# shamanDevel/IsosurfaceSuperresolution

Hardware: AMD Instinct MI355X
Metric: frames/sec (render+4×SR) at 256³→1080p, 1/2/4/8 GPU; PSNR vs ref (higher is better)
Workload: dtype f32 (fp32 tensors and accumulation; each product as three fp16 MFMAs on split operands, error vs fp64 = the fp32 kernels')

## Files before the change

### include/isr_sr_kernels.h

```cpp
#ifndef ISR_SR_KERNELS_H
#define ISR_SR_KERNELS_H

#ifdef __cplusplus
extern "C" {
#endif

#define ISR_ACT_NONE 0
#define ISR_ACT_RELU 1
#define ISR_ACT_LEAKY 2
#define ISR_ACT_GATE 3

int isrConvCinPad(int Cin);
int isrConvCoutPad(int Cout);

int isrConvPrepareWeights(const float* w, float* wprep, int Cout, int Cin, int transpose_flip, void* stream);

int isrConv3x3Forward(const float* x, const float* wprep, const float* bias, const float* residual, float* y,
                      int N, int Cin, int H, int W, int Cout, int act, float slope, int upsample2x, void* stream);

int isrConv3x3ForwardStrided(const float* x, const float* wprep, const float* bias, const float* residual, float* y,
                             int N, int Cin, int H, int W, int Cout, int act, float slope, int upsample2x,
                             long long xPlane, long long xImage, long long yPlane, long long yImage,
                             long long rPlane, long long rImage, void* stream);

int isrConvSmallCinPad(int Cin);
long long isrConvSmallWeightFloats(int Cin);
int isrConvSmallPrepare(const float* w, const float* bias, float* w8, float* bias8, int Cout, int Cin, void* stream);
int isrConv3x3SmallCout(const float* x, const float* w8, const float* bias8, const float* residual, float* y,
                        int N, int Cin, int H, int W, int Cout, int act, float slope, void* stream);
int isrConv3x3SmallCoutStrided(const float* x, const float* w8, const float* bias8, const float* residual, float* y,
                               int N, int Cin, int H, int W, int Cout, int act, float slope,
                               long long xPlane, long long xImage, void* stream);

long long isrConvSplitWeightBytes(int Cin, int Cout);
int isrConvSplitPrepare(const float* w, void* wq, int Cout, int Cin, void* stream);
int isrConvSplitPrepareManyMax(void);
int isrConvSplitPrepareMany(int n, const float* const* w, void* const* wqForward, void* const* wqBackward, const int* cout, const int* cin, void* stream);
int isrConv3x3ForwardSplit(const float* x, const void* wq, const float* bias, const float* residual, float* y,
                           int N, int Cin, int H, int W, int Cout, int act, float slope, int upsample2x,
                           long long xPlane, long long xImage, long long yPlane, long long yImage,
                           long long rPlane, long long rImage, void* stream);

long long isrConvF16WeightBytes(int Cin, int Cout);
int isrConvF16Prepare(const float* w, void* wq, int Cout, int Cin, void* stream);
int isrConv3x3ForwardF16(const float* x, const void* wq, const float* bias, const float* residual, float* y,
                         int N, int Cin, int H, int W, int Cout, int act, float slope, int upsample2x,
                         long long xPlane, long long xImage, long long yPlane, long long yImage,
                         long long rPlane, long long rImage, void* stream);
int isrConvBf16Prepare(const float* w, void* wq, int Cout, int Cin, void* stream);
int isrConv3x3ForwardBf16(const float* x, const void* wq, const float* bias, const float* residual, float* y,
                          int N, int Cin, int H, int W, int Cout, int act, float slope, int upsample2x,
                          long long xPlane, long long xImage, long long yPlane, long long yImage,
                          long long rPlane, long long rImage, void* stream);
int isrConvF16SupportsUpsample(long long x_address, int Win, long long xPlane, long long xImage);

long long isrConvWeightGradWorkspace(int N, int Cin, int H, int W, int Cout);
int isrConv3x3WeightGrad(const float* x, const float* gz, float* dw, float* db, void* workspace,
                         int N, int Cin, int H, int W, int Cout, void* stream);

int isrConvWeightGradMaxSegments(void);
int isrConv3x3WeightGradSegments(const float* const* xs, const float* const* gzs, int segments, float* dw, float* db, void* workspace,
                                 int N, int Cin, int H, int W, int Cout, void* stream);
int isrConv3x3WeightGradSegmentsSplit(const float* const* xs, const float* const* gzs, int segments, float* dw, float* db, void* workspace,
                                      int N, int Cin, int H, int W, int Cout, void* stream);
void isrSetMaxSlots(void* words, int capacity);
int isrTakeMaxSlotWords(void);
int isrConv3x3WeightGradSegmentsSplitMax(const float* const* xs, const float* const* gzs, const void* const* gzmax, int maxWords, int segments,
                                         float* dw, float* db, void* workspace, int N, int Cin, int H, int W, int Cout, void* stream);
void isrSetWeightGradAccumulate(int bits);
int isrConv3x3WeightGradSegmentsBf16(const float* const* xs, const float* const* gzs, int segments, float* dw, float* db, void* workspace,
                                     int N, int Cin, int H, int W, int Cout, void* stream);

int isrUpsample2xForward(const float* x, float* y, long long planes, int h, int w, void* stream);
int isrUpsample2xBackward(const float* gy, float* gx, long long planes, int h, int w, void* stream);

int isrReconResidualForward(const float* y, const float* x, float* out, int N, int Cout, int Cin, int k, int h, int w, void* stream);
int isrReconResidualBackward(const float* gy, float* gx, int N, int Cout, int Cin, int k, int h, int w, void* stream);

long long isrLossUnshadedWorkspace(void);
int isrLossUnshadedForward(const float* gt, const float* pred, const float* prev, int N, int H, int W, int pad,
                           const float* weights15, unsigned enabled, const float* shading12, float ao_strength, int inverse_ao,
                           void* workspace, float* values16, void* stream);
int isrLossUnshadedBackward(const float* gt, const float* pred, const float* prev, int N, int H, int W, int pad,
                            const float* weights15, unsigned enabled, const float* shading12, float ao_strength, int inverse_ao,
                            const float* gvalues16, float* gpred, float* gprev, void* stream);

int isrRecurrentInputForward(const float* prev_raw, const float* input, const float* flow, float* net_input, float* warped,
                             int B, int h, int w, long long inputBatchStride, long long flowBatchStride, void* stream);
int isrRecurrentInputBackward(const float* prev_raw, const float* flow, const float* g_net_input, const float* g_warped,
                              float* scratch, float* g_prev_raw, int B, int h, int w, long long flowBatchStride, void* stream);

int isrAdamFlatStep(float* params, const float* grads, float* exp_avg, float* exp_avg_sq, long long n, const float* lr_dev, float lr,
                    float beta1, float beta2, float eps, float* step, void* stream);

int isrActBackward(const float* gy, const float* y, float* gz, long long count, int act, float slope, void* stream);

int isrAssembleInput(const float* gbuffer_hwc12, const float* flow_filled, const float* prev_high, float* net_input,
                     int h, int w, int init_mode, int ao_inverted, void* stream);
int isrAssembleInputRows(const float* gbuffer_hwc12, const float* flow_filled, const float* prev_high, float* net_input,
                         int h, int w, int init_mode, int ao_inverted, int row0, int row1, void* stream);
int isrAssembleInputRect(const float* gbuffer_hwc12, const float* flow_filled, const float* prev_high, float* net_input,
                         int h, int w, int init_mode, int ao_inverted, int row0, int row1, int col0, int col1, void* stream);
int isrAssembleInputPacked(const float* gbuffer_hwc12, const float* flow_filled, const float* prev_high, float* net_input,
                           int h, int w, int init_mode, int ao_inverted, void* trunk_workspace, void* stream);

long long isrFlowFillWorkspace(int h, int w);
int isrFlowFill(const float* gbuffer_hwc12, float* flow_out, void* workspace, int h, int w, void* stream);
int isrFlowFillEx(const float* gbuffer_hwc12, float* flow_out, void* workspace, int h, int w, int threads, void* stream);
int isrFlowFillOneSupported(int h, int w);
int isrFlowFillOne(const float* gbuffer_hwc12, float* flow_out, void* workspace, int h, int w, void* stream);
void isrSetFlowFillErrorWord(unsigned* word);

int isrFinishFrame(const float* raw, const float* net_input, float* next_prev, float* rgb, int h, int w,
                   const float* shading24, int exponent, float ao_strength, int inverse_ao, int enable_specular, void* stream);

int isrConvSmallFinishFrame(const float* x, const float* w8, const float* bias8, const float* net_input, float* next_prev, float* rgb,
                            int Cin, int h, int w, long long xPlane, const float* shading24, int exponent, float ao_strength,
                            int inverse_ao, int enable_specular, void* stream);

int isrConv3x3ForwardSplitPacked(const float* x, const void* wq, const float* bias, void* ps, int Cin, int H, int W, int Cout,
                                 int act, float slope, int upsample2x, long long xPlane, long long psPlane, void* stream);

int isrConv3x3ForwardSplitFromPacked(const void* xps, const void* wq, const float* bias, const float* residual, void* y, int packed_out,
                                     int Cin, int H, int W, int Cout, int act, float slope, long long xpsPlane, long long yPlane, long long rPlane,
                                     void* stream);

int isrTrunkDataflowMaxTiles(void);
long long isrTrunkDataflowWorkspaceBytes(int cin0, int H, int W);
int isrTrunkDataflowSupported(const float* x, int cin0, int H, int W, long long xPlane, long long plane);
int isrTrunkDataflow(const float* x, int cin0, long long xPlane, float* y, long long plane, const void* const* wq,
                     const float* const* bias, int nblocks, int H, int W, void* workspace, void* stream);
int isrTrunkDataflowInputLayout(int cin0, int H, int W, long long* offsets3, int* groups0, int* tiles);
int isrTrunkDataflowPrepacked(int cin0, float* y, long long plane, const void* const* wq, const float* const* bias, int nblocks, int H, int W,
                              void* workspace, void* stream);
void isrSetTrunkErrorWord(unsigned* word);

int isrResBlockSmallSupported(int N, int H, int W);
int isrResBlockSmall(const float* x, const void* wa, const float* ba, const float* gate, const void* wb, const float* bb, float* z, float* y,
                     int N, int H, int W, void* zmax, void* ymax, void* stream);

long long isrResBlockSplitWorkspaceBytes(void);
int isrResBlockSplitSupported(const float* x, int H, int W, long long xPlane, long long yPlane);
int isrResBlockSplit(const float* x, const void* wq1, const float* bias1, const void* wq2, const float* bias2, float* y, void* workspace,
                     int H, int W, long long xPlane, long long yPlane, void* stream);

long long isrConvTailWeightBytes(void);
long long isrConvTailWorkspaceBytes(int h, int w);
int isrConvTailPrepare(const float* w8, void* wz, void* stream);
int isrConvTailSupported(const float* x, int h, int w, long long xPlane);
int isrConvTailFinishFrame(const float* x, const void* wq6, const float* bias6, const void* wz, const float* bias8, void* workspace,
                           const float* net_input, float* next_prev, float* rgb, int h, int w, long long xPlane,
                           const float* shading24, int exponent, float ao_strength, int inverse_ao, int enable_specular, void* stream);
int isrConvTailFinishFramePacked(const void* xps, const void* wq6, const float* bias6, const void* wz, const float* bias8, void* workspace,
                                 const float* net_input, float* next_prev, float* rgb, int h, int w, long long xpsPlane,
                                 const float* shading24, int exponent, float ao_strength, int inverse_ao, int enable_specular, void* stream);

long long isrConvUpsPhaseWeightBytes(void);
long long isrConvUpsPhaseScratchBytes(void);
int isrConvUpsPhasePrepare(const float* w, void* wq, void* scratch, void* stream);
int isrConvUpsPhaseSupported(int Cin, int Cout, int h, int wd, long long xpsPlane, long long psPlane);
int isrConvUpsPhase(const void* xps, const void* wq, const float* w, const float* bias, void* ps, int h, int wd, int act, float slope,
                    long long xpsPlane, long long psPlane, void* stream);
int isrPackSplit(const float* x, void* ps, int C, int H, int W, long long xPlane, long long psPlane, void* stream);
int isrTrunkDataflowPackedResult(int cin0, int H, int W, long long* offsetBytes, long long* planeUnits);
void isrSetTrunkPackedResult(int on);
void isrSetTrunkRows(int rows);

int isrProfileEnable(int on);
int isrProfileCount(void);
int isrProfileGet(int i, int* variant, double* flops, float* ms);

#ifdef __cplusplus
}
#endif
#endif
```

### isosurfacesuperresolution_amd/csrc/sr_conv_trunk.hip

```cpp
#include "sr_diag.h"
#include <cstdlib>
#include <cstring>

#include "sr_split_common.h"

namespace {

#ifndef T16_EARLY_PATCH
#define T16_EARLY_PATCH 5
#endif
constexpr int T16_H = 16, T16_W = 32, T16_THREADS = 512, T16_WAVES = 8;
constexpr int P16_H = T16_H + 2, P16_W = T16_W + 2, P16_PIX = P16_H * P16_W;
constexpr int P16_PART = 2 * P16_PIX;
constexpr int P16_UNITS = 2 * P16_PART;
constexpr int P16_SUBS = (P16_PIX + 63) / 64;
constexpr int T16_LDS_UNITS = 2 * P16_UNITS + 2 * S_WUNITS;
constexpr int T16_LDS_BYTES = T16_LDS_UNITS * 16 + 2 * 64 * 4 + 64;
constexpr int T16_MAX_LAYERS = 24;

struct Trunk16Params {
    const u32x4* wq[T16_MAX_LAYERS]; const float* bias[T16_MAX_LAYERS];
    const char* ws;
    unsigned xpsOff, fpsOff, tpsOff;
    int groups0;
    float* y; int yPlane;
    unsigned* done;
    unsigned* error;
    unsigned* absmax;
    int H, W, plane, tilesX, tilesY, layers;
    ISR_DIAG_MEMBER(int, dbg, 0);
    ISR_DIAG_MEMBER(int, faultTile, -1);
    int lastPacked;
    unsigned long long timeoutTicks;
    ISR_DIAG_MEMBER(unsigned long long*, stamps, nullptr);
};

template <typename T>
__device__ __forceinline__ T* trunk16_uniform(T* q)
{
    const unsigned long long v = (unsigned long long)q;
    const unsigned lo = __builtin_amdgcn_readfirstlane((unsigned)v), hi = __builtin_amdgcn_readfirstlane((unsigned)(v >> 32));
    return (T*)(((unsigned long long)hi << 32) | lo);
}

[[maybe_unused]] int g_trunk_dbg = 0;
[[maybe_unused]] unsigned long long* g_trunk_stamps = nullptr;
unsigned* g_trunk_error_word = nullptr;
[[maybe_unused]] int g_trunk_fault_tile = -1;
unsigned long long g_trunk_timeout_ticks = 5000000ull;

typedef __attribute__((address_space(3))) char t16_lds_char;

#pragma clang diagnostic push
#pragma clang diagnostic ignored "-Winline-asm"
template <bool COHERENT = false>
__device__ __forceinline__ void trunk16_dma16(const void* base, unsigned voff, unsigned ldsaddr)
{
    ldsaddr = __builtin_amdgcn_readfirstlane(ldsaddr);
    if (COHERENT)
        asm volatile("s_mov_b32 m0, %0\n\ts_nop 0\n\tglobal_load_lds_dwordx4 %1, %2 sc1" :: "s"(ldsaddr), "v"(voff), "s"(base) : "m0");
    else
        asm volatile("s_mov_b32 m0, %0\n\ts_nop 0\n\tglobal_load_lds_dwordx4 %1, %2" :: "s"(ldsaddr), "v"(voff), "s"(base) : "m0");
}
template <bool COHERENT = true>
__device__ __forceinline__ void trunk16_dma16_masked(const void* base, unsigned voff, unsigned ldsaddr, unsigned long long mask)
{
    ldsaddr = __builtin_amdgcn_readfirstlane(ldsaddr);
    unsigned long long saved;
    if (COHERENT)
        asm volatile("s_mov_b64 %0, exec\n\ts_mov_b64 exec, %4\n\ts_mov_b32 m0, %1\n\ts_nop 0\n\tglobal_load_lds_dwordx4 %2, %3 sc1\n\ts_mov_b64 exec, %0"
                     : "=&s"(saved) : "s"(ldsaddr), "v"(voff), "s"(base), "s"(mask) : "m0");
    else
        asm volatile("s_mov_b64 %0, exec\n\ts_mov_b64 exec, %4\n\ts_mov_b32 m0, %1\n\ts_nop 0\n\tglobal_load_lds_dwordx4 %2, %3\n\ts_mov_b64 exec, %0"
                     : "=&s"(saved) : "s"(ldsaddr), "v"(voff), "s"(base), "s"(mask) : "m0");
}
__device__ __forceinline__ void trunk16_dma4(const void* base, unsigned voff, unsigned ldsaddr)
{
    ldsaddr = __builtin_amdgcn_readfirstlane(ldsaddr);
    asm volatile("s_mov_b32 m0, %0\n\ts_nop 0\n\tglobal_load_lds_dword %1, %2" :: "s"(ldsaddr), "v"(voff), "s"(base) : "m0");
}
#pragma clang diagnostic pop

template <int ROWS>
struct Trunk16Operands { f16x8 a0h, a0l, a1h, a1l, bh[ROWS], bo[ROWS]; };

template <int ROWS>
__device__ __forceinline__ Trunk16Operands<ROWS> trunk16_operands(const u32x4* wl, const u32x4* bl, int tap)
{
    const int dy = tap / 3, dx = tap - dy * 3;
    Trunk16Operands<ROWS> o;
    o.a0h = __builtin_bit_cast(f16x8, wl[tap * 128]);
    o.a0l = __builtin_bit_cast(f16x8, wl[S_WPART + tap * 128]);
    o.a1h = __builtin_bit_cast(f16x8, wl[tap * 128 + 32]);
    o.a1l = __builtin_bit_cast(f16x8, wl[S_WPART + tap * 128 + 32]);
#pragma unroll
    for (int r = 0; r < ROWS; ++r) {
        o.bh[r] = __builtin_bit_cast(f16x8, bl[(r + dy) * P16_W + dx]);
        o.bo[r] = __builtin_bit_cast(f16x8, bl[P16_PART + (r + dy) * P16_W + dx]);
    }
    return o;
}

struct Trunk16NoMid { __device__ __forceinline__ void operator()(int, int) const {} };

template <int ROWS, typename Between, typename Mid = Trunk16NoMid>
__device__ __forceinline__ void trunk16_kstep(f32x16 (&acc)[2][ROWS], const u32x4* wl, const u32x4* bl, Between between, Mid mid = Mid())
{
    Trunk16Operands<ROWS> cur = trunk16_operands<ROWS>(wl, bl, 0);
#pragma unroll
    for (int tap = 0; tap < 9; ++tap) {
        Trunk16Operands<ROWS> nxt = cur;
        if (tap < 8) {
            nxt = trunk16_operands<ROWS>(wl, bl, tap + 1);
            __builtin_amdgcn_sched_barrier(0);
        }
        const f16x8 a0s = cur.a0h * (_Float16)0.00048828125f;
        const f16x8 a1s = cur.a1h * (_Float16)0.00048828125f;
        if (ROWS == 2) {
#pragma unroll
            for (int r = 0; r < ROWS; ++r) {
                acc[0][r] = mfma16(cur.a0l, cur.bh[r], acc[0][r]);
                acc[0][r] = mfma16(a0s, cur.bo[r], acc[0][r]);
                acc[0][r] = mfma16(cur.a0h, cur.bh[r], acc[0][r]);
                mid(tap, r);
                acc[1][r] = mfma16(cur.a1l, cur.bh[r], acc[1][r]);
                acc[1][r] = mfma16(a1s, cur.bo[r], acc[1][r]);
                acc[1][r] = mfma16(cur.a1h, cur.bh[r], acc[1][r]);
            }
        } else {
#pragma unroll
            for (int r = 0; r < ROWS; ++r) { acc[0][r] = mfma16(cur.a0l, cur.bh[r], acc[0][r]); acc[1][r] = mfma16(cur.a1l, cur.bh[r], acc[1][r]); }
            mid(tap, 0);
#pragma unroll
            for (int r = 0; r < ROWS; ++r) { acc[0][r] = mfma16(a0s, cur.bo[r], acc[0][r]); acc[1][r] = mfma16(a1s, cur.bo[r], acc[1][r]); }
            mid(tap, 1);
#pragma unroll
            for (int r = 0; r < ROWS; ++r) { acc[0][r] = mfma16(cur.a0h, cur.bh[r], acc[0][r]); acc[1][r] = mfma16(cur.a1h, cur.bh[r], acc[1][r]); }
        }
        between(tap);
        cur = nxt;
    }
}

struct Trunk16Lane {
    unsigned poff[P16_SUBS];
    unsigned live, centre;
};

__device__ __forceinline__ Trunk16Lane trunk16_lane_setup(const Trunk16Params& p, int oy0, int ox0, int lane)
{
    Trunk16Lane t;
    t.live = 0u; t.centre = 0u;
#pragma unroll
    for (int sub = 0; sub < P16_SUBS; ++sub) {
        const int off = sub * 64 + lane;
        const int r = off / P16_W, c = off - r * P16_W;
        const int iy = oy0 + r - 1, ix = ox0 + c - 1;
        t.poff[sub] = (unsigned)(((unsigned)iy < (unsigned)p.H && (unsigned)ix < (unsigned)p.W) ? iy * p.W + ix : p.H * p.W) * 16u;
        if (off < P16_PIX) t.live |= 1u << sub;
        if (r >= 1 && r <= T16_H && c >= 1 && c <= T16_W) t.centre |= 1u << sub;
    }
    return t;
}

template <bool HALO_ONLY>
__device__ __forceinline__ void trunk16_patch_run(int sub, const char* plane, unsigned pbufRole, const Trunk16Lane& t)
{
    const unsigned take = HALO_ONLY ? (t.live & ~t.centre) : t.live;
    if (take & (1u << sub)) trunk16_dma16<true>(plane, t.poff[sub], pbufRole + (unsigned)sub * 1024u);
}

template <int KIND, bool LAST, bool DIAG, int ROWS>
__device__ __forceinline__ void trunk16_epilogue(const Trunk16Params& p, f32x16 (&acc)[2][ROWS], f32x16 (&F)[2][ROWS], unsigned& mag, float unscale,
                                                 const float* biasl, const char* out, unsigned planeBytes, int oy0, int ox0, int wave, int j, int h,
                                                 u32x4* pk0, u32x4* pk1)
{
    const rsrc_t prs = __builtin_amdgcn_make_buffer_rsrc(const_cast<char*>(LAST ? reinterpret_cast<const char*>(p.y) : out), 0,
                                                         LAST ? (int)((size_t)64 * p.yPlane * 4) : (int)(16u * planeBytes), 0x00020000);
    const rsrc_t qrs = __builtin_amdgcn_make_buffer_rsrc(const_cast<char*>(out), 0, (int)(16u * planeBytes), 0x00020000);
    const int ox = ox0 + j;
#pragma unroll
    for (int r = 0; r < ROWS; ++r) {
        const int oy = oy0 + wave * ROWS + r;
        const bool inside = oy < p.H && ox < p.W && !(DIAG && (p.dbg & 4));
        const unsigned voff = !inside ? BAD_OFFSET : LAST ? (unsigned)(oy * p.W + ox + 4 * h * p.yPlane) * 4u
                                                          : (unsigned)(oy * p.W + ox) * 16u + 8u * (unsigned)h;
        const int row = wave * ROWS + r;
        const bool ring = row == 0 || row == T16_H - 1 || j == 0 || j == T16_W - 1;
        const unsigned voffRing = ring ? voff : BAD_OFFSET;
        const bool live = oy < p.H && ox < p.W;
        u32x2* const c0 = reinterpret_cast<u32x2*>(pk0 + (row + 1) * P16_W + j + 1) + h;
        u32x2* const c1 = reinterpret_cast<u32x2*>(pk1 + (row + 1) * P16_W + j + 1) + h;
#pragma unroll
        for (int cb = 0; cb < 2; ++cb) {
#pragma unroll
            for (int gi = 0; gi < 4; ++gi) {
                const float4 b4 = *reinterpret_cast<const float4*>(biasl + cb * 32 + 8 * gi + 4 * h);
                const float bv[4] = {b4.x, b4.y, b4.z, b4.w};
                f16x4 th, tl;
#pragma unroll
                for (int e = 0; e < 4; ++e) {
                    float v = acc[cb][r][4 * gi + e] * unscale + bv[e];
                    if (KIND != 2) v = v > 0.f ? v : 0.f;
                    else v += F[cb][r][4 * gi + e];
                    if (KIND != 1) F[cb][r][4 * gi + e] = v;
                    if (inside) mag = isr_umax(mag, isr_mag(v));
                    if (LAST) __builtin_amdgcn_raw_buffer_store_b32(__builtin_bit_cast(unsigned, v), prs, (int)voff, (cb * 32 + 8 * gi + e) * p.yPlane * 4, 0);
                    _Float16 a, b;
                    split16x(v, a, b);
                    th[e] = a; tl[e] = b;
                }
                if (LAST) {
                    const int g = cb * 4 + gi;
                    const unsigned vq = (inside && p.lastPacked) ? (unsigned)(oy * p.W + ox) * 16u + 8u * (unsigned)h : BAD_OFFSET;
                    __builtin_amdgcn_raw_buffer_store_b64(__builtin_bit_cast(u32x2, th), qrs, (int)vq, g * planeBytes, 0);
                    __builtin_amdgcn_raw_buffer_store_b64(__builtin_bit_cast(u32x2, tl), qrs, (int)vq, (8 + g) * planeBytes, 0);
                } else {
                    const int g = cb * 4 + gi;
                    const unsigned vo = cb == 0 ? voffRing : voff;
                    __builtin_amdgcn_raw_buffer_store_b64(__builtin_bit_cast(u32x2, th), prs, (int)vo, g * planeBytes, 16);
                    __builtin_amdgcn_raw_buffer_store_b64(__builtin_bit_cast(u32x2, tl), prs, (int)vo, (8 + g) * planeBytes, 16);
                    if (cb == 0) {
                        const u32x2 zero2 = {0u, 0u};
                        u32x2* const c = (gi < 2 ? c0 : c1) + (gi & 1) * (P16_PIX * 2);
                        c[0] = live ? __builtin_bit_cast(u32x2, th) : zero2;
                        c[P16_PART * 2] = live ? __builtin_bit_cast(u32x2, tl) : zero2;
                    }
                }
            }
        }
    }
}

template <bool DIAG, int ROWS, bool LINE = (ROWS == 4)>
__global__ __launch_bounds__(64 * T16_H / ROWS) void trunk_dataflow_kernel(const Trunk16Params p)
{
    constexpr int WAVES = T16_H / ROWS;
    const int dbg = DIAG ? p.dbg : 0;
    extern __shared__ u32x4 lds[];
    u32x4* const pbuf0 = lds;
    u32x4* const wbuf0 = lds + 2 * P16_UNITS;
    float* const biasl0 = reinterpret_cast<float*>(lds + T16_LDS_UNITS);
    int* const flags = reinterpret_cast<int*>(biasl0 + 128);
    const unsigned ldsBase = (unsigned)(uintptr_t)(t16_lds_char*)lds;
    const unsigned pAddr = ldsBase, wAddr = ldsBase + 2 * P16_UNITS * 16, bAddr = ldsBase + T16_LDS_UNITS * 16;
    const int tid = threadIdx.x, lane = tid & 63;
    const int wave = __builtin_amdgcn_readfirstlane(tid >> 6);
    const int j = lane & 31, h = lane >> 5;
    const int ntiles = p.tilesX * p.tilesY;
    int tile;
    {
        const int nwg = gridDim.x, q = nwg >> 3, r = nwg & 7, xcd = blockIdx.x & 7;
        tile = (xcd < r ? xcd * (q + 1) : r * (q + 1) + (xcd - r) * q) + (blockIdx.x >> 3);
    }
    if (tile >= ntiles) return;
    const int tx = tile % p.tilesX, ty = tile / p.tilesX;
    const int oy0 = ty * T16_H, ox0 = tx * T16_W;
    const unsigned long long deadline = __builtin_amdgcn_s_memrealtime() + p.timeoutTicks;
    const Trunk16Lane lanes = trunk16_lane_setup(p, oy0, ox0, lane);

    f32x16 F[2][ROWS];
#pragma unroll
    for (int cb = 0; cb < 2; ++cb)
#pragma unroll
        for (int r = 0; r < ROWS; ++r)
#pragma unroll
            for (int i = 0; i < 16; ++i) F[cb][r][i] = 0.0f;
    unsigned mag = 0u;
    int gk = 0;

    const char* const ws = trunk16_uniform(p.ws);
    const unsigned planeBytes = (unsigned)p.plane * 16u;
    const bool dmaX = !(dbg & 2), dmaW = !(dbg & 16);
    const u32x4* wq = trunk16_uniform(p.wq[0]);
    auto stage_bias = [&](int l, const float* b) {
        if (wave != WAVES - 1) return;
        if (b) trunk16_dma4(b, (unsigned)lane * 4u, bAddr + (unsigned)(l & 1) * 256u);
        else biasl0[(l & 1) * 64 + lane] = 0.0f;
    };
    const bool wrole = WAVES == 4 || wave < 4, prole = WAVES == 4 || wave >= 4;
    const int rpart = (wave & 3) >> 1, rsel = wave & 1;
    const unsigned wdstRole = (unsigned)(rpart * S_WPART + rsel * 64) * 16u;
    const unsigned pdstRole = (unsigned)((rpart * 2 + rsel) * P16_PIX) * 16u;
    const unsigned wlane = (unsigned)lane * 16u;
    auto weight_tap = [&](int tap, const u32x4* image, int ksteps_, int ks, unsigned wbuf) {
        trunk16_dma16(image + 1 + (size_t)(tap * ksteps_ + ks) * 256 + rpart * 128 + rsel * 64, wlane, wbuf + wdstRole + (unsigned)tap * 2048u);
    };
    auto patch_plane = [&](const char* tensor, int groups_, int ks) {
        return tensor + (size_t)(rpart * groups_ + 2 * ks + rsel) * planeBytes;
    };
    stage_bias(0, trunk16_uniform(p.bias[0]));
    if (wrole && dmaW) {
#pragma unroll
        for (int tap = 0; tap < 9; ++tap) weight_tap(tap, wq, p.groups0 >> 1, 0, wAddr);
    }
    if (prole && dmaX) {
        const char* const plane = patch_plane(ws + p.xpsOff, p.groups0, 0);
#pragma unroll
        for (int sub = 0; sub < P16_SUBS; ++sub) trunk16_patch_run<false>(sub, plane, pAddr + pdstRole, lanes);
    }

#pragma unroll 1
    for (int l = 0; l < p.layers; ++l) {
        const int kind = l == 0 ? 0 : (l & 1) ? 1 : 2;
        const int groups = l == 0 ? p.groups0 : 8, ksteps = groups >> 1;
        const char* const tin = ws + (l == 0 ? p.xpsOff : (l & 1) ? p.fpsOff : p.tpsOff);
        const char* const tout = ws + ((l & 1) ? p.tpsOff : p.fpsOff);
        const bool last = l + 1 == p.layers;
        const u32x4* const wqNext = last ? nullptr : trunk16_uniform(p.wq[l + 1]);
        const float* const biasNext = last ? nullptr : trunk16_uniform(p.bias[l + 1]);
        auto lap = [&](int slot) {
            if (DIAG && p.stamps && tid == 0) p.stamps[((size_t)tile * p.layers + l) * 8 + slot] = __builtin_amdgcn_s_memrealtime();
        };
        lap(0);
        if (l > 0) {
            if (!(dbg & 8)) {
                if (tid == 0) flags[0] = 0;
                __syncthreads();
                if (tid < 9 && tid != 4) {
                    const int ny = ty + tid / 3 - 1, nx = tx + tid % 3 - 1;
                    if ((unsigned)ny < (unsigned)p.tilesY && (unsigned)nx < (unsigned)p.tilesX) {
                        const unsigned* f = p.done + ny * p.tilesX + nx;
                        while (__hip_atomic_load(f, __ATOMIC_RELAXED, __HIP_MEMORY_SCOPE_AGENT) < (unsigned)l) {
                            __builtin_amdgcn_s_sleep(2);
                            if (__builtin_amdgcn_s_memrealtime() > deadline) { flags[0] = 1; break; }
                        }
                    }
                }
                __syncthreads();
                if (flags[0]) {
                    if (tid == 0) atomicMax(p.error, (unsigned)(1 + l));
                    return;
                }
            }
            lap(1);
            if (dmaX && prole) {
                const char* const plane = patch_plane(tin, groups, 0);
#pragma unroll
                for (int sub = 0; sub < P16_SUBS; ++sub) trunk16_patch_run<true>(sub, plane, pAddr + (unsigned)(gk & 1) * (P16_UNITS * 16) + pdstRole, lanes);
            }
        }
        f32x16 acc[2][ROWS];
#pragma unroll
        for (int cb = 0; cb < 2; ++cb)
#pragma unroll
            for (int r = 0; r < ROWS; ++r)
#pragma unroll
                for (int i = 0; i < 16; ++i) acc[cb][r][i] = 0.0f;
#pragma unroll 1
        for (int ks = 0; ks < ksteps; ++ks, ++gk) {
            asm volatile("s_waitcnt vmcnt(0)" ::: "memory");
            __syncthreads();
            if (ks == 0) lap(2);
            const int cur = gk & 1, nxt = cur ^ 1;
            const u32x4* const pcur = pbuf0 + cur * P16_UNITS;
            const u32x4* const wcur = wbuf0 + cur * S_WUNITS;
            const unsigned pnxt = pAddr + (unsigned)nxt * (P16_UNITS * 16), wnxt = wAddr + (unsigned)nxt * (S_WUNITS * 16);
            const bool more = ks + 1 < ksteps;
            const u32x4* const wimg = more ? wq : wqNext;
            const int wks = more ? ks + 1 : 0, wksteps = more ? ksteps : 4;
            const bool wany = dmaW && (more || !last), pany = dmaX && more;
            const bool haloOnly = l > 0 && ks == 0;
            const char* const pplane = patch_plane(tin, groups, ks + 1);
            auto between = [&](int tap) {
                if (wrole) {
                    if (wany) weight_tap(tap, wimg, wksteps, wks, wnxt);
                }
                if (prole) {
                    if (pany) {
                        if (T16_EARLY_PATCH) {
#pragma unroll
                            for (int q = 0; q < T16_EARLY_PATCH; ++q) {
                                const int run = T16_EARLY_PATCH * tap + q;
                                if (run < P16_SUBS) {
                                    if (haloOnly) trunk16_patch_run<true>(run, pplane, pnxt + pdstRole, lanes);
                                    else trunk16_patch_run<false>(run, pplane, pnxt + pdstRole, lanes);
                                }
                            }
                        } else if (haloOnly) {
                            trunk16_patch_run<true>(tap, pplane, pnxt + pdstRole, lanes);
                            if (tap == 8) trunk16_patch_run<true>(9, pplane, pnxt + pdstRole, lanes);
                        } else {
                            trunk16_patch_run<false>(tap, pplane, pnxt + pdstRole, lanes);
                            if (tap == 8) trunk16_patch_run<false>(9, pplane, pnxt + pdstRole, lanes);
                        }
                    } else if (!more && !last && tap == 0) stage_bias(l + 1, biasNext);
                }
            };
            if (ROWS == 2 && (dbg & 32)) {
                const f16x8 a = __builtin_bit_cast(f16x8, wcur[h * 64 + j]), b = __builtin_bit_cast(f16x8, pcur[h * P16_PIX + j]);
                if (dbg & 64) {
#pragma unroll
                    for (int t = 0; t < 9; ++t) {
                        const Trunk16Operands<ROWS> o = trunk16_operands<ROWS>(wcur + h * 64 + j, pcur + h * P16_PIX + (wave * ROWS) * P16_W + j, t);
                        asm volatile("" :: "v"(o.a0h), "v"(o.a0l), "v"(o.a1h), "v"(o.a1l));
#pragma unroll
                        for (int r = 0; r < ROWS; ++r) asm volatile("" :: "v"(o.bh[r]), "v"(o.bo[r]));
#pragma unroll
                        for (int q = 0; q < 3; ++q)
#pragma unroll
                            for (int cb = 0; cb < 2; ++cb)
#pragma unroll
                                for (int r = 0; r < ROWS; ++r) acc[cb][r] = mfma16(a, b, acc[cb][r]);
                        between(t);
                    }
                } else {
#pragma unroll
                    for (int t = 0; t < 27; ++t)
#pragma unroll
                        for (int cb = 0; cb < 2; ++cb)
#pragma unroll
                            for (int r = 0; r < ROWS; ++r) acc[cb][r] = mfma16(a, b, acc[cb][r]);
#pragma unroll
                    for (int t = 0; t < 9; ++t) between(t);
                }
            } else if (LINE && !(dbg & 1)) {
                if (!more && !last) stage_bias(l + 1, biasNext);
                const u32x4* const wsrc = (wany ? wimg : wq) + 1 + (size_t)wks * 256 + rpart * 128 + rsel * 64;
                const size_t wtap = (size_t)(wany ? wksteps : ksteps) * 256;
                const unsigned wdst = wnxt + wdstRole;
                const unsigned takeBits = (l > 0 && ks == 0) ? (lanes.live & ~lanes.centre) : lanes.live;
                const unsigned long long pmask = __builtin_amdgcn_ballot_w64(pany && prole), wmask = __builtin_amdgcn_ballot_w64(wany && wrole);
                auto mid = [&](int tap, int q) {
                    if (q == 0) trunk16_dma16_masked<false>(wsrc + tap * wtap, wlane, wdst + (unsigned)tap * 2048u, wmask);
                    else {
#pragma unroll
                        for (int qq = 0; qq < T16_EARLY_PATCH; ++qq) {
                            const int run = T16_EARLY_PATCH * tap + qq;
                            if (run < P16_SUBS)
                                trunk16_dma16_masked(pplane, lanes.poff[run], pnxt + pdstRole + (unsigned)run * 1024u, __builtin_amdgcn_ballot_w64((takeBits >> run) & 1u) & pmask);
                        }
                    }
                };
                trunk16_kstep<ROWS>(acc, wcur + h * 64 + j, pcur + h * P16_PIX + (wave * ROWS) * P16_W + j, [](int) {}, mid);
            } else if (!(dbg & 1)) {
                trunk16_kstep<ROWS>(acc, wcur + h * 64 + j, pcur + h * P16_PIX + (wave * ROWS) * P16_W + j, between);
            } else {
#pragma unroll
                for (int t = 0; t < 9; ++t) between(t);
            }
        }
        __syncthreads();
        lap(3);
        {
            const float unscale = reinterpret_cast<const float*>(wq)[1];
            const float* const biasl = biasl0 + (l & 1) * 64;
            u32x4* const pk0 = pbuf0 + (gk & 1) * P16_UNITS;
            u32x4* const pk1 = pbuf0 + ((gk + 1) & 1) * P16_UNITS;
            if (last) {
                if (kind == 0) trunk16_epilogue<0, true, DIAG, ROWS>(p, acc, F, mag, unscale, biasl, tout, planeBytes, oy0, ox0, wave, j, h, pk0, pk1);
                else trunk16_epilogue<2, true, DIAG, ROWS>(p, acc, F, mag, unscale, biasl, tout, planeBytes, oy0, ox0, wave, j, h, pk0, pk1);
            } else if (kind == 0) trunk16_epilogue<0, false, DIAG, ROWS>(p, acc, F, mag, unscale, biasl, tout, planeBytes, oy0, ox0, wave, j, h, pk0, pk1);
            else if (kind == 1) trunk16_epilogue<1, false, DIAG, ROWS>(p, acc, F, mag, unscale, biasl, tout, planeBytes, oy0, ox0, wave, j, h, pk0, pk1);
            else trunk16_epilogue<2, false, DIAG, ROWS>(p, acc, F, mag, unscale, biasl, tout, planeBytes, oy0, ox0, wave, j, h, pk0, pk1);
        }
        lap(4);
        asm volatile("s_waitcnt vmcnt(0)" ::: "memory");
        __syncthreads();
        if (tid == 0 && tile != p.faultTile) __hip_atomic_store(p.done + tile, (unsigned)(l + 1), __ATOMIC_RELAXED, __HIP_MEMORY_SCOPE_AGENT);
        wq = wqNext;
        lap(5);
    }
    isr_range_note(p.absmax, mag);
}

template <int KIND, bool LAST>
__device__ __forceinline__ void trunk_mt_epilogue(const Trunk16Params& p, f32x16 (&acc)[2][2], unsigned& mag, float unscale, const float* biasl,
                                                  const char* out, unsigned planeBytes, int oy0, int ox0, int wave, int j, int h)
{
    const rsrc_t prs = __builtin_amdgcn_make_buffer_rsrc(const_cast<char*>(out), 0, (int)(16u * planeBytes), 0x00020000);
    const rsrc_t yrs = __builtin_amdgcn_make_buffer_rsrc(reinterpret_cast<char*>(p.y), 0, (int)((size_t)64 * p.yPlane * 4), 0x00020000);
    const int ox = ox0 + j;
#pragma unroll
    for (int r = 0; r < 2; ++r) {
        const int oy = oy0 + wave * 2 + r;
        const bool inside = oy < p.H && ox < p.W;
        const unsigned voff = !inside ? BAD_OFFSET : (unsigned)(oy * p.W + ox) * 16u + 8u * (unsigned)h;
        const unsigned yoff = !inside ? BAD_OFFSET : (unsigned)(oy * p.W + ox + 4 * h * p.yPlane) * 4u;
        float fold[2][16];
        if (KIND == 2) {
#pragma unroll
            for (int cb = 0; cb < 2; ++cb)
#pragma unroll
                for (int i = 0; i < 16; ++i)
                    fold[cb][i] = __builtin_bit_cast(float, __builtin_amdgcn_raw_buffer_load_b32(yrs, (int)yoff, (cb * 32 + 8 * (i >> 2) + (i & 3)) * p.yPlane * 4, 16));
        }
#pragma unroll
        for (int cb = 0; cb < 2; ++cb) {
#pragma unroll
            for (int gi = 0; gi < 4; ++gi) {
                const float4 b4 = *reinterpret_cast<const float4*>(biasl + cb * 32 + 8 * gi + 4 * h);
                const float bv[4] = {b4.x, b4.y, b4.z, b4.w};
                f16x4 th, tl;
#pragma unroll
                for (int e = 0; e < 4; ++e) {
                    float v = acc[cb][r][4 * gi + e] * unscale + bv[e];
                    if (KIND != 2) v = v > 0.f ? v : 0.f;
                    else v += fold[cb][4 * gi + e];
                    if (inside) mag = isr_umax(mag, isr_mag(v));
                    if (KIND != 1) __builtin_amdgcn_raw_buffer_store_b32(__builtin_bit_cast(unsigned, v), yrs, (int)yoff, (cb * 32 + 8 * gi + e) * p.yPlane * 4, LAST ? 0 : 16);
                    _Float16 a, b;
                    split16x(v, a, b);
                    th[e] = a; tl[e] = b;
                }
                {
                    const int g = cb * 4 + gi;
                    const unsigned vq = (LAST && !p.lastPacked) ? BAD_OFFSET : voff;
                    __builtin_amdgcn_raw_buffer_store_b64(__builtin_bit_cast(u32x2, th), prs, (int)vq, g * planeBytes, LAST ? 0 : 16);
                    __builtin_amdgcn_raw_buffer_store_b64(__builtin_bit_cast(u32x2, tl), prs, (int)vq, (8 + g) * planeBytes, LAST ? 0 : 16);
                }
            }
        }
    }
}

__global__ __launch_bounds__(T16_THREADS) void trunk_mt_kernel(const Trunk16Params p)
{
    extern __shared__ u32x4 lds[];
    u32x4* const pbuf0 = lds;
    u32x4* const wbuf0 = lds + 2 * P16_UNITS;
    float* const biasl0 = reinterpret_cast<float*>(lds + T16_LDS_UNITS);
    int* const flags = reinterpret_cast<int*>(biasl0 + 128);
    const unsigned ldsBase = (unsigned)(uintptr_t)(t16_lds_char*)lds;
    const unsigned pAddr = ldsBase, wAddr = ldsBase + 2 * P16_UNITS * 16, bAddr = ldsBase + T16_LDS_UNITS * 16;
    const int tid = threadIdx.x, lane = tid & 63;
    const int wave = __builtin_amdgcn_readfirstlane(tid >> 6);
    const int j = lane & 31, h = lane >> 5;
    const int ntiles = p.tilesX * p.tilesY;
    const int nwg = gridDim.x;
    int slot;
    {
        const int q = nwg >> 3, r = nwg & 7, xcd = blockIdx.x & 7;
        slot = (xcd < r ? xcd * (q + 1) : r * (q + 1) + (xcd - r) * q) + (blockIdx.x >> 3);
    }
    if (slot >= ntiles) return;
    const unsigned long long waitTicks = p.timeoutTicks * (unsigned long long)((ntiles + nwg - 1) / nwg);
    unsigned mag = 0u;
    int gk = 0;
    const char* const ws = trunk16_uniform(p.ws);
    const unsigned planeBytes = (unsigned)p.plane * 16u;
    const bool wrole = wave < 4;
    const int rpart = (wave & 3) >> 1, rsel = wave & 1;
    const unsigned wdstRole = (unsigned)(rpart * S_WPART + rsel * 64) * 16u;
    const unsigned pdstRole = (unsigned)((rpart * 2 + rsel) * P16_PIX) * 16u;
    const unsigned wlane = (unsigned)lane * 16u;
    auto weight_tap = [&](int tap, const u32x4* image, int ksteps_, int ks, unsigned wbuf) {
        trunk16_dma16(image + 1 + (size_t)(tap * ksteps_ + ks) * 256 + rpart * 128 + rsel * 64, wlane, wbuf + wdstRole + (unsigned)tap * 2048u);
    };
    auto patch_plane = [&](const char* tensor, int groups_, int ks) {
        return tensor + (size_t)(rpart * groups_ + 2 * ks + rsel) * planeBytes;
    };
#pragma unroll 1
    for (int l = 0; l < p.layers; ++l) {
        const int kind = l == 0 ? 0 : (l & 1) ? 1 : 2;
        const int groups = l == 0 ? p.groups0 : 8, ksteps = groups >> 1;
        const char* const tin = ws + (l == 0 ? p.xpsOff : (l & 1) ? p.fpsOff : p.tpsOff);
        const char* const tout = ws + ((l & 1) ? p.tpsOff : p.fpsOff);
        const bool last = l + 1 == p.layers;
        const u32x4* const wq = trunk16_uniform(p.wq[l]);
        const float* const bias = trunk16_uniform(p.bias[l]);
        const float unscale = reinterpret_cast<const float*>(wq)[1];
        bool staged = false;
        int owed = -1;
        Trunk16Lane lanes = trunk16_lane_setup(p, (slot / p.tilesX) * T16_H, (slot % p.tilesX) * T16_W, lane);
#pragma unroll 1
        for (int tile = slot; tile < ntiles; tile += nwg) {
            const int tx = tile % p.tilesX, ty = tile / p.tilesX;
            const int oy0 = ty * T16_H, ox0 = tx * T16_W;
            const int tnext = tile + nwg;
            const int txn = tnext % p.tilesX, tyn = tnext / p.tilesX;
            bool ahead = tnext < ntiles;
            if (l > 0) {
                if (tid == 0) { flags[0] = 0; flags[1] = 0; }
                __syncthreads();
                if (tid < 9) {
                    const int ny = ty + tid / 3 - 1, nx = tx + tid % 3 - 1;
                    if ((unsigned)ny < (unsigned)p.tilesY && (unsigned)nx < (unsigned)p.tilesX) {
                        const unsigned* f = p.done + ny * p.tilesX + nx;
                        if (__hip_atomic_load(f, __ATOMIC_RELAXED, __HIP_MEMORY_SCOPE_AGENT) < (unsigned)l) {
                            const unsigned long long deadline = __builtin_amdgcn_s_memrealtime() + waitTicks;
                            do {
                                __builtin_amdgcn_s_sleep(2);
                                if (__builtin_amdgcn_s_memrealtime() > deadline) { flags[0] = 1; break; }
                            } while (__hip_atomic_load(f, __ATOMIC_RELAXED, __HIP_MEMORY_SCOPE_AGENT) < (unsigned)l);
                        }
                    }
                } else if (tid >= 64 && tid < 73 && ahead) {
                    const int q = tid - 64, ny = tyn + q / 3 - 1, nx = txn + q % 3 - 1;
                    if ((unsigned)ny < (unsigned)p.tilesY && (unsigned)nx < (unsigned)p.tilesX &&
                        __hip_atomic_load(p.done + ny * p.tilesX + nx, __ATOMIC_RELAXED, __HIP_MEMORY_SCOPE_AGENT) < (unsigned)l) flags[1] = 1;
                }
                __syncthreads();
                if (flags[0]) {
                    if (tid == 0) atomicMax(p.error, (unsigned)(1 + l));
                    return;
                }
                ahead = ahead && !__builtin_amdgcn_readfirstlane(flags[1]);
            }
            const Trunk16Lane lanesNext = trunk16_lane_setup(p, tyn * T16_H, txn * T16_W, lane);
            if (!staged) {
                if (tile == slot && wave == T16_WAVES - 1) {
                    if (bias) trunk16_dma4(bias, (unsigned)lane * 4u, bAddr);
                    else biasl0[lane] = 0.0f;
                }
                if (wrole) {
#pragma unroll
                    for (int tap = 0; tap < 9; ++tap) weight_tap(tap, wq, ksteps, 0, wAddr + (unsigned)(gk & 1) * (S_WUNITS * 16));
                } else {
                    const char* const plane = patch_plane(tin, groups, 0);
#pragma unroll
                    for (int sub = 0; sub < P16_SUBS; ++sub) trunk16_patch_run<false>(sub, plane, pAddr + (unsigned)(gk & 1) * (P16_UNITS * 16) + pdstRole, lanes);
                }
            }
            f32x16 acc[2][2];
#pragma unroll
            for (int cb = 0; cb < 2; ++cb)
#pragma unroll
                for (int r = 0; r < 2; ++r)
#pragma unroll
                    for (int i = 0; i < 16; ++i) acc[cb][r][i] = 0.0f;
#pragma unroll 1
            for (int ks = 0; ks < ksteps; ++ks, ++gk) {
                asm volatile("s_waitcnt vmcnt(0)" ::: "memory");
                __syncthreads();
                if (owed >= 0) {
                    if (tid == 0 && owed != p.faultTile) __hip_atomic_store(p.done + owed, (unsigned)(l + 1), __ATOMIC_RELAXED, __HIP_MEMORY_SCOPE_AGENT);
                    owed = -1;
                }
                const int cur = gk & 1, nxt = cur ^ 1;
                const u32x4* const pcur = pbuf0 + cur * P16_UNITS;
                const u32x4* const wcur = wbuf0 + cur * S_WUNITS;
                const unsigned pnxt = pAddr + (unsigned)nxt * (P16_UNITS * 16), wnxt = wAddr + (unsigned)nxt * (S_WUNITS * 16);
                const bool more = ks + 1 < ksteps;
                const char* const pplane = patch_plane(tin, groups, more ? ks + 1 : 0);
                auto between = [&](int tap) {
                    if (more) {
                        if (wrole) weight_tap(tap, wq, ksteps, ks + 1, wnxt);
                        else {
#pragma unroll
                            for (int q = 0; q < T16_EARLY_PATCH; ++q)
                                if (T16_EARLY_PATCH * tap + q < P16_SUBS) trunk16_patch_run<false>(T16_EARLY_PATCH * tap + q, pplane, pnxt + pdstRole, lanes);
                        }
                    } else if (ahead) {
                        if (wrole) weight_tap(tap, wq, ksteps, 0, wnxt);
                        else {
#pragma unroll
                            for (int q = 0; q < T16_EARLY_PATCH; ++q)
                                if (T16_EARLY_PATCH * tap + q < P16_SUBS) trunk16_patch_run<false>(T16_EARLY_PATCH * tap + q, pplane, pnxt + pdstRole, lanesNext);
                        }
                    }
                };
                trunk16_kstep<2>(acc, wcur + h * 64 + j, pcur + h * P16_PIX + (wave * 2) * P16_W + j, between);
            }
            __syncthreads();
            if (last) {
                if (kind == 0) trunk_mt_epilogue<0, true>(p, acc, mag, unscale, biasl0, tout, planeBytes, oy0, ox0, wave, j, h);
                else trunk_mt_epilogue<2, true>(p, acc, mag, unscale, biasl0, tout, planeBytes, oy0, ox0, wave, j, h);
            } else if (kind == 0) trunk_mt_epilogue<0, false>(p, acc, mag, unscale, biasl0, tout, planeBytes, oy0, ox0, wave, j, h);
            else if (kind == 1) trunk_mt_epilogue<1, false>(p, acc, mag, unscale, biasl0, tout, planeBytes, oy0, ox0, wave, j, h);
            else trunk_mt_epilogue<2, false>(p, acc, mag, unscale, biasl0, tout, planeBytes, oy0, ox0, wave, j, h);
            if (tnext < ntiles) owed = tile;
            else {
                asm volatile("s_waitcnt vmcnt(0)" ::: "memory");
                __syncthreads();
                if (tid == 0 && tile != p.faultTile) __hip_atomic_store(p.done + tile, (unsigned)(l + 1), __ATOMIC_RELAXED, __HIP_MEMORY_SCOPE_AGENT);
            }
            staged = ahead;
            lanes = lanesNext;
        }
    }
    isr_range_note(p.absmax, mag);
}

__global__ __launch_bounds__(256) void trunk_pack_input_kernel(const float* __restrict__ x, int cin, long long xPlane, int npix, u32x4* __restrict__ ps,
                                                               int groups, u32x4* __restrict__ fps, u32x4* __restrict__ tps,
                                                               unsigned* __restrict__ done, int ntiles)
{
    const int pix = blockIdx.x * 256 + threadIdx.x, g = blockIdx.y;
    if (blockIdx.x == 0 && g == 0)
        for (int i = threadIdx.x; i < ntiles; i += 256) done[i] = 0u;
    const size_t plane = ((size_t)npix + 8) & ~(size_t)7;
    const u32x4 zero = {0u, 0u, 0u, 0u};
    if (blockIdx.x == 0 && threadIdx.x < 2) {
        if (g < groups) ps[(size_t)(threadIdx.x * groups + g) * plane + npix] = zero;
        if (g < 8) {
            fps[(size_t)(threadIdx.x * 8 + g) * plane + npix] = zero;
            tps[(size_t)(threadIdx.x * 8 + g) * plane + npix] = zero;
        }
    }
    if (pix >= npix || g >= groups) return;
    f16x8 hi, lo;
#pragma unroll
    for (int e = 0; e < 8; ++e) {
        const int c = g * 8 + e;
        const float v = c < cin ? x[(size_t)c * xPlane + pix] : 0.0f;
        _Float16 a, b;
        split16x(v, a, b);
        hi[e] = a; lo[e] = b;
    }
    ps[(size_t)g * plane + pix] = __builtin_bit_cast(u32x4, hi);
    ps[(size_t)(groups + g) * plane + pix] = __builtin_bit_cast(u32x4, lo);
}

inline long long align256(long long v) { return (v + 255) & ~255LL; }

struct Trunk16Layout { long long header, xps, fps, tps, total; int tiles, groups0; };

Trunk16Layout trunk16_layout(int cin0, int H, int W)
{
    Trunk16Layout o;
    o.tiles = ((W + T16_W - 1) / T16_W) * ((H + T16_H - 1) / T16_H);
    o.groups0 = 2 * ((cin0 + 15) / 16);
    const long long plane = ((long long)H * W + 8) & ~7LL;
    o.header = 0;
    o.xps = align256(16 + (long long)(o.tiles + 1) * 4);
    o.fps = o.xps + align256(2LL * o.groups0 * plane * 16);
    o.tps = o.fps + align256(2LL * 8 * plane * 16);
    o.total = o.tps + align256(2LL * 8 * plane * 16);
    return o;
}

}

extern "C" {

#ifdef ISR_DIAG
void isrDebugSetTrunkAblation(int mask) { g_trunk_dbg = mask & 127; }
void isrDebugSetTrunkStampBuffer(unsigned long long* stamps) { g_trunk_stamps = stamps; }
int isrDebugTrunkState(void);
void isrDebugSetTrunkFault(int tile, unsigned long long timeoutTicks)
{
    g_trunk_fault_tile = tile;
    g_trunk_timeout_ticks = timeoutTicks ? timeoutTicks : 5000000ull;
}
#endif
void isrSetTrunkErrorWord(unsigned* word) { g_trunk_error_word = word; }

static int g_trunk_mt = isr_diag_env_int("ISR_TRUNK_MT", 1);
static int g_trunk_rows = (getenv("ISR_TRUNK_ROWS") && atoi(getenv("ISR_TRUNK_ROWS")) == 4) ? 4 : 2;
void isrSetTrunkRows(int rows) { g_trunk_rows = rows == 4 ? 4 : 2; }
#ifdef ISR_DIAG
void isrDebugSetTrunkMultiTile(int mode) { g_trunk_mt = mode; }
int isrDebugTrunkState(void)
{
    return g_trunk_dbg | ((g_trunk_fault_tile >= 0 || g_trunk_timeout_ticks != 5000000ull) ? 128 : 0) | (g_trunk_stamps ? 256 : 0) | (g_trunk_mt != 1 ? 512 : 0);
}
#endif

int isrTrunkDataflowMaxTiles(void)
{
    int dev = 0, cus = 0;
    (void)hipGetDevice(&dev);
    if (hipDeviceGetAttribute(&cus, hipDeviceAttributeMultiprocessorCount, dev) != hipSuccess || cus <= 0) cus = 256;
    return cus;
}

long long isrTrunkDataflowWorkspaceBytes(int cin0, int H, int W)
{
    if (H <= 0 || W <= 0 || cin0 <= 0) return -1;
    return trunk16_layout(cin0, H, W).total;
}

static int g_trunk_last_packed = 0;
void isrSetTrunkPackedResult(int on) { g_trunk_last_packed = on ? 1 : 0; }

int isrTrunkDataflowPackedResult(int cin0, int H, int W, long long* offsetBytes, long long* planeUnits)
{
    if (H <= 0 || W <= 0 || cin0 <= 0 || !offsetBytes || !planeUnits) return -1;
    *offsetBytes = trunk16_layout(cin0, H, W).fps;
    *planeUnits = ((long long)H * W + 8) & ~7LL;
    return 0;
}

int isrTrunkDataflowSupported(const float* x, int cin0, int H, int W, long long xPlane, long long plane)
{
    if (!x || H <= 0 || W <= 0 || cin0 <= 0 || cin0 > 1024) return 0;
    if (xPlane < (long long)H * W || plane < (long long)H * W || plane * 64 * 4 > 0x7fffffffLL) return 0;
    if (trunk16_layout(cin0, H, W).total > 0xffffffffLL || ((long long)H * W + 8) * 16 * 16 > 0x7fffffffLL) return 0;
    const long long tiles = (long long)((W + T16_W - 1) / T16_W) * ((H + T16_H - 1) / T16_H);
    return (tiles <= isrTrunkDataflowMaxTiles() || (g_trunk_mt && tiles <= 65535)) ? 1 : 0;
}

int isrTrunkDataflowInputLayout(int cin0, int H, int W, long long* offsets3, int* groups0, int* tiles)
{
    if (H <= 0 || W <= 0 || cin0 <= 0 || !offsets3 || !groups0 || !tiles) return -1;
    const Trunk16Layout lay = trunk16_layout(cin0, H, W);
    if (lay.total > 0xffffffffLL) return -3;
    offsets3[0] = lay.xps; offsets3[1] = lay.fps; offsets3[2] = lay.tps;
    *groups0 = lay.groups0; *tiles = lay.tiles;
    return 0;
}

static int trunk_dataflow_launch(const float* x, bool prepacked, int cin0, long long xPlane, float* y, long long plane, const void* const* wq,
                                 const float* const* bias, int nblocks, int H, int W, void* workspace, void* stream);

int isrTrunkDataflow(const float* x, int cin0, long long xPlane, float* y, long long plane, const void* const* wq,
                     const float* const* bias, int nblocks, int H, int W, void* workspace, void* stream)
{
    return trunk_dataflow_launch(x, false, cin0, xPlane, y, plane, wq, bias, nblocks, H, W, workspace, stream);
}

int isrTrunkDataflowPrepacked(int cin0, float* y, long long plane, const void* const* wq, const float* const* bias, int nblocks, int H, int W,
                              void* workspace, void* stream)
{
    return trunk_dataflow_launch(nullptr, true, cin0, (long long)H * W, y, plane, wq, bias, nblocks, H, W, workspace, stream);
}

static int trunk_dataflow_launch(const float* x, bool prepacked, int cin0, long long xPlane, float* y, long long plane, const void* const* wq,
                                 const float* const* bias, int nblocks, int H, int W, void* workspace, void* stream)
{
    unsigned* const rangeFlag = isr_take_range_flag();
    if ((!x && !prepacked) || !y || !wq || !bias || !workspace || nblocks < 0 || 1 + 2 * nblocks > T16_MAX_LAYERS || cin0 <= 0) return -1;
    if (!isrTrunkDataflowSupported(prepacked ? y : x, cin0, H, W, xPlane, plane) || ((uintptr_t)workspace & 255)) return -3;
    const Trunk16Layout lay = trunk16_layout(cin0, H, W);
    char* ws = (char*)workspace;
    u32x4* xps = (u32x4*)(ws + lay.xps);
    Trunk16Params p;
    std::memset(&p, 0, sizeof(p));
    const int layers = 1 + 2 * nblocks;
    for (int l = 0; l < layers; ++l) {
        if (!wq[l]) return -1;
        p.wq[l] = (const u32x4*)wq[l]; p.bias[l] = bias[l];
    }
    p.xpsOff = (unsigned)lay.xps; p.fpsOff = (unsigned)lay.fps; p.tpsOff = (unsigned)lay.tps; p.groups0 = lay.groups0;
    p.y = y; p.yPlane = (int)plane;
    p.H = H; p.W = W; p.plane = (int)(((long long)H * W + 8) & ~7LL); p.layers = layers;
    p.tilesX = (W + T16_W - 1) / T16_W; p.tilesY = (H + T16_H - 1) / T16_H;
    const int ntiles = p.tilesX * p.tilesY;
    p.ws = ws; p.done = (unsigned*)(ws + 16); p.error = g_trunk_error_word ? g_trunk_error_word : p.done + ntiles;
    p.absmax = rangeFlag;
    ISR_DIAG_SET(p.dbg, g_trunk_dbg); ISR_DIAG_SET(p.stamps, g_trunk_stamps);
    p.timeoutTicks = g_trunk_timeout_ticks;
    ISR_DIAG_SET(p.faultTile, g_trunk_fault_tile);
    p.lastPacked = g_trunk_last_packed;
    hipStream_t s = (hipStream_t)stream;
    static bool attr = false;
    if (!attr) {
        (void)hipFuncSetAttribute((const void*)trunk_dataflow_kernel<false, 2>, hipFuncAttributeMaxDynamicSharedMemorySize, T16_LDS_BYTES);
        (void)hipFuncSetAttribute((const void*)trunk_dataflow_kernel<false, 4>, hipFuncAttributeMaxDynamicSharedMemorySize, T16_LDS_BYTES);
#ifdef ISR_DIAG
        (void)hipFuncSetAttribute((const void*)trunk_dataflow_kernel<true, 2>, hipFuncAttributeMaxDynamicSharedMemorySize, T16_LDS_BYTES);
        (void)hipFuncSetAttribute((const void*)trunk_dataflow_kernel<true, 4>, hipFuncAttributeMaxDynamicSharedMemorySize, T16_LDS_BYTES);
#endif
        (void)hipFuncSetAttribute((const void*)trunk_mt_kernel, hipFuncAttributeMaxDynamicSharedMemorySize, T16_LDS_BYTES);
        attr = true;
    }
#ifdef ISR_DIAG
    const bool diag = p.dbg != 0 || p.stamps != nullptr;
#endif
    const int npix = H * W;
    if (!prepacked)
        ISR_LAUNCH_PROFILED(ISR_VARIANT_TRUNK_PACK, trunk_pack_input_kernel, dim3((unsigned)((npix + 255) / 256), (unsigned)(lay.groups0 > 8 ? lay.groups0 : 8)), dim3(256), 0, s,
                            x, cin0, xPlane, npix, xps, lay.groups0, (u32x4*)(ws + lay.fps), (u32x4*)(ws + lay.tps), p.done, ntiles);
    hipEvent_t e0 = nullptr, e1 = nullptr;
    const int cus = isrTrunkDataflowMaxTiles();
    const bool mt = g_trunk_mt == 2 || ntiles > cus;
    isr_profile_record(mt ? ISR_VARIANT_SPLIT_TRUNK_MT : ISR_VARIANT_SPLIT_TRUNK, 2.0 * 9 * 64 * ((double)cin0 + 2.0 * nblocks * 64) * (double)H * W, &e0, &e1);
    const dim3 grid((unsigned)(((ntiles + 7) / 8) * 8)), block(T16_THREADS);
    if (mt) {
        const int round8 = ((ntiles + 7) / 8) * 8;
        const dim3 mgrid((unsigned)(round8 < cus ? round8 : cus));
        if (e0 || e1) hipExtLaunchKernelGGL(trunk_mt_kernel, mgrid, block, T16_LDS_BYTES, s, e0, e1, 0, p);
        else hipLaunchKernelGGL(trunk_mt_kernel, mgrid, block, T16_LDS_BYTES, s, p);
    } else if (g_trunk_rows == 4) {
        const dim3 block4(256);
#ifdef ISR_DIAG
        if (diag) {
            if (e0 || e1) hipExtLaunchKernelGGL((trunk_dataflow_kernel<true, 4>), grid, block4, T16_LDS_BYTES, s, e0, e1, 0, p);
            else hipLaunchKernelGGL((trunk_dataflow_kernel<true, 4>), grid, block4, T16_LDS_BYTES, s, p);
        } else
#endif
        if (e0 || e1) hipExtLaunchKernelGGL((trunk_dataflow_kernel<false, 4>), grid, block4, T16_LDS_BYTES, s, e0, e1, 0, p);
        else hipLaunchKernelGGL((trunk_dataflow_kernel<false, 4>), grid, block4, T16_LDS_BYTES, s, p);
    } else {
#ifdef ISR_DIAG
        if (diag) {
            if (e0 || e1) hipExtLaunchKernelGGL((trunk_dataflow_kernel<true, 2>), grid, block, T16_LDS_BYTES, s, e0, e1, 0, p);
            else hipLaunchKernelGGL((trunk_dataflow_kernel<true, 2>), grid, block, T16_LDS_BYTES, s, p);
        } else
#endif
        if (e0 || e1) hipExtLaunchKernelGGL((trunk_dataflow_kernel<false, 2>), grid, block, T16_LDS_BYTES, s, e0, e1, 0, p);
        else hipLaunchKernelGGL((trunk_dataflow_kernel<false, 2>), grid, block, T16_LDS_BYTES, s, p);
    }
    return hipGetLastError() == hipSuccess ? 0 : -2;
}

}
```

Baseline: 615.6.

## Rebuild centre patch of odd trunk layers from register-resident residual instead of DMA

Measured after the change: 618.6 (median of 6 runs). About the same (+0.5%).

```diff
diff --git a/include/isr_sr_kernels.h b/include/isr_sr_kernels.h
--- a/include/isr_sr_kernels.h
+++ b/include/isr_sr_kernels.h
@@ -165,6 +165,7 @@
 int isrTrunkDataflowPackedResult(int cin0, int H, int W, long long* offsetBytes, long long* planeUnits);
 void isrSetTrunkPackedResult(int on);
 void isrSetTrunkRows(int rows);
+int isrTrunkRows(void);
 
 int isrProfileEnable(int on);
 int isrProfileCount(void);
diff --git a/isosurfacesuperresolution_amd/csrc/sr_conv_trunk.hip b/isosurfacesuperresolution_amd/csrc/sr_conv_trunk.hip
--- a/isosurfacesuperresolution_amd/csrc/sr_conv_trunk.hip
+++ b/isosurfacesuperresolution_amd/csrc/sr_conv_trunk.hip
@@ -217,7 +217,7 @@
                     __builtin_amdgcn_raw_buffer_store_b64(__builtin_bit_cast(u32x2, tl), qrs, (int)vq, (8 + g) * planeBytes, 0);
                 } else {
                     const int g = cb * 4 + gi;
-                    const unsigned vo = cb == 0 ? voffRing : voff;
+                    const unsigned vo = (cb == 0 || KIND != 1) ? voffRing : voff;
                     __builtin_amdgcn_raw_buffer_store_b64(__builtin_bit_cast(u32x2, th), prs, (int)vo, g * planeBytes, 16);
                     __builtin_amdgcn_raw_buffer_store_b64(__builtin_bit_cast(u32x2, tl), prs, (int)vo, (8 + g) * planeBytes, 16);
                     if (cb == 0) {
@@ -228,6 +228,33 @@
                     }
                 }
             }
+        }
+    }
+}
+
+template <int GI0, int ROWS>
+__device__ __forceinline__ void trunk16_centre_from_F(const Trunk16Params& p, const f32x16 (&F)[2][ROWS], u32x4* pk, int oy0, int ox0, int wave, int j, int h)
+{
+    const int ox = ox0 + j;
+    const u32x2 zero2 = {0u, 0u};
+#pragma unroll
+    for (int r = 0; r < ROWS; ++r) {
+        const int row = wave * ROWS + r;
+        const bool live = oy0 + row < p.H && ox < p.W;
+        u32x2* const c = reinterpret_cast<u32x2*>(pk + (row + 1) * P16_W + j + 1) + h;
+#pragma unroll
+        for (int g = 0; g < 2; ++g) {
+            f16x4 th, tl;
+#pragma unroll
+            for (int e = 0; e < 4; ++e) {
+                float v = F[1][r][4 * (GI0 + g) + e];
+                asm volatile("" : "+v"(v));
+                _Float16 a, b;
+                split16x(v, a, b);
+                th[e] = a; tl[e] = b;
+            }
+            c[g * (P16_PIX * 2)] = live ? __builtin_bit_cast(u32x2, th) : zero2;
+            c[g * (P16_PIX * 2) + P16_PART * 2] = live ? __builtin_bit_cast(u32x2, tl) : zero2;
         }
     }
 }
@@ -360,7 +387,7 @@
             const u32x4* const wimg = more ? wq : wqNext;
             const int wks = more ? ks + 1 : 0, wksteps = more ? ksteps : 4;
             const bool wany = dmaW && (more || !last), pany = dmaX && more;
-            const bool haloOnly = l > 0 && ks == 0;
+            const bool haloOnly = l > 0 && (ks == 0 || (l & 1));
             const char* const pplane = patch_plane(tin, groups, ks + 1);
             auto between = [&](int tap) {
                 if (wrole) {
@@ -419,7 +446,7 @@
                 const u32x4* const wsrc = (wany ? wimg : wq) + 1 + (size_t)wks * 256 + rpart * 128 + rsel * 64;
                 const size_t wtap = (size_t)(wany ? wksteps : ksteps) * 256;
                 const unsigned wdst = wnxt + wdstRole;
-                const unsigned takeBits = (l > 0 && ks == 0) ? (lanes.live & ~lanes.centre) : lanes.live;
+                const unsigned takeBits = haloOnly ? (lanes.live & ~lanes.centre) : lanes.live;
                 const unsigned long long pmask = __builtin_amdgcn_ballot_w64(pany && prole), wmask = __builtin_amdgcn_ballot_w64(wany && wrole);
                 auto mid = [&](int tap, int q) {
                     if (q == 0) trunk16_dma16_masked<false>(wsrc + tap * wtap, wlane, wdst + (unsigned)tap * 2048u, wmask);
@@ -438,6 +465,11 @@
             } else {
 #pragma unroll
                 for (int t = 0; t < 9; ++t) between(t);
+            }
+            if (l & 1) {
+                u32x4* const pk = pbuf0 + nxt * P16_UNITS;
+                if (ks == 1) trunk16_centre_from_F<0, ROWS>(p, F, pk, oy0, ox0, wave, j, h);
+                else if (ks == 2) trunk16_centre_from_F<2, ROWS>(p, F, pk, oy0, ox0, wave, j, h);
             }
         }
         __syncthreads();
@@ -739,6 +771,7 @@
 static int g_trunk_mt = isr_diag_env_int("ISR_TRUNK_MT", 1);
 static int g_trunk_rows = (getenv("ISR_TRUNK_ROWS") && atoi(getenv("ISR_TRUNK_ROWS")) == 4) ? 4 : 2;
 void isrSetTrunkRows(int rows) { g_trunk_rows = rows == 4 ? 4 : 2; }
+int isrTrunkRows(void) { return g_trunk_rows; }
 #ifdef ISR_DIAG
 void isrDebugSetTrunkMultiTile(int mode) { g_trunk_mt = mode; }
 int isrDebugTrunkState(void)
```
